# jneem/nnnoiseless

Hardware: AMD Instinct MI355X
Metric: 480-sample frames/sec (whole node) at N concurrent streams (higher is better)
Workload: dtype f32; 1 GPU; configs[2]: 65536 concurrent streams on one GPU, built-in weights.rnn, GRU as batched MFMA GEMM, synthetic 48 kHz sine+noise, 48 frame(s) per stream per step; parity=oracle pinned by the reference's golden pair (built-in model), model=built-in weights.rnn, boundary_format=f32 planar (process_frame's own), streams_per_gpu=65536, streams_total=65536, inputs_ready=True, schedule=stages, lanes=2, parallelism=streams sharded x1, one process per GPU, no data-path collective

## Files before the change

include/nnn_batch.h:

```cpp
#ifndef NNN_BATCH_H
#define NNN_BATCH_H

#include <stddef.h>
#include <stdint.h>

#ifdef __cplusplus
extern "C" {
#endif

typedef struct nnn_batch nnn_batch;
#ifndef RNNOISE_H
typedef struct RNNModel RNNModel;
#endif

#define NNN_FRAME_SIZE 480

RNNModel *nnn_model_from_bytes(const uint8_t *bytes, size_t len);
RNNModel *nnn_model_default(void);
long nnn_convert_rnnoise_text(const char *text, size_t len, uint8_t *out, size_t cap);
RNNModel *nnn_model_from_rnnoise_text(const char *text, size_t len);
void nnn_model_free(RNNModel *m);
RNNModel *nnn_model_clone(const RNNModel *m);
void nnn_model_shape(const RNNModel *m, int32_t shape[12]);

// ... 77 lines not shown
                             const nnn_pcm_layout *layout, void *hip_stream);
int nnn_batch_synthesize_device(nnn_batch *b, const float *d_gains, const float *d_vad, void *d_out, int n_frames,
                                const nnn_pcm_layout *layout, void *hip_stream);
int nnn_batch_analyze_host(nnn_batch *b, const void *in, float *features, int32_t *silence, int n_frames, const nnn_pcm_layout *layout);
int nnn_batch_synthesize_host(nnn_batch *b, const float *gains, const float *vad, void *out, int n_frames, const nnn_pcm_layout *layout);
int nnn_batch_pending_frames(const nnn_batch *b);
int nnn_batch_vad_device(nnn_batch *b, const void *d_in, float *d_vad, int n_frames, const nnn_pcm_layout *layout, void *hip_stream);
int nnn_batch_vad_host(nnn_batch *b, const void *in, float *vad, int n_frames, const nnn_pcm_layout *layout);
int nnn_batch_network_device(nnn_batch *b, const float *d_features, const int32_t *d_silence, float *d_gains, float *d_vad, int n_frames,
                             void *hip_stream);
int nnn_batch_network_host(nnn_batch *b, const float *features, const int32_t *silence, float *gains, float *vad, int n_frames);
int nnn_batch_synchronize(nnn_batch *b);
int nnn_batch_fault(const nnn_batch *b);
int nnn_batch_debug_withhold_flag(nnn_batch *b, int frames_ahead);
int nnn_batch_debug_schedule(nnn_batch *b, int n_frames, int32_t *out, size_t cap);
int nnn_batch_debug_host_plan(nnn_batch *b, int n_frames, const nnn_pcm_layout *layout, int has_vad, int64_t out[8]);

enum nnn_tap {
    NNN_TAP_FILTERED = 0,
    NNN_TAP_XLP,
    NNN_TAP_AC,
    NNN_TAP_LPC2,
    NNN_TAP_XCORR1,
    NNN_TAP_BEST1,
    NNN_TAP_XCORR2C,
    NNN_TAP_PITCH_SEARCH,
    NNN_TAP_PITCH,
    NNN_TAP_PITCH_GAIN,
    NNN_TAP_X,
    NNN_TAP_P,
// ... 40 lines not shown
```

nnnoiseless_amd/_ffi.py:

```python
import ctypes as C
import os

import numpy as np

FRAME_SIZE = 480

TAPS = ["filtered", "xlp", "ac", "lpc2", "xcorr1", "best1", "xcorr2c", "pitch_search", "pitch", "pitch_gain",
        "X", "P", "ex", "ep", "exp", "features", "silence", "g_raw", "g", "vad", "branch"]

BATCH_SYMBOLS = [
    "nnn_model_from_bytes", "nnn_model_default", "nnn_model_free", "nnn_model_clone", "nnn_model_shape",
    "nnn_convert_rnnoise_text", "nnn_model_from_rnnoise_text",
    "nnn_batch_create", "nnn_batch_create_grouped", "nnn_batch_destroy", "nnn_batch_num_streams", "nnn_batch_reset",
    "nnn_batch_process_device", "nnn_batch_process_host", "nnn_batch_process_pcm_device", "nnn_batch_process_pcm_host",
    "nnn_batch_synchronize", "nnn_batch_clone", "nnn_batch_state_bytes", "nnn_batch_save_state", "nnn_batch_load_state",
    "nnn_batch_set_taps", "nnn_batch_set_schedule", "nnn_batch_set_inputs_ready", "nnn_debug_activations",
    "nnn_tap_info", "nnn_batch_read_tap", "nnn_batch_set_profiling", "nnn_batch_num_kernels",
    "nnn_batch_kernel_name", "nnn_batch_read_kernel_times", "nnn_batch_set_graph", "nnn_batch_set_pipeline", "nnn_batch_read_stamps",
    "nnn_host_alloc", "nnn_host_free", "nnn_last_error", "nnn_batch_fault", "nnn_batch_debug_withhold_flag", "nnn_batch_debug_schedule", "nnn_batch_debug_host_plan", "nnn_batch_set_frame_log",
    "nnn_batch_create_opts", "nnn_batch_max_group_frames", "nnn_batch_device_bytes", "nnn_batch_set_back_end", "nnn_device_local_cpulist",
    "nnn_batch_reset_streams", "nnn_batch_export_streams", "nnn_batch_import_streams", "nnn_batch_export_streams_device",
    "nnn_batch_import_streams_device", "nnn_batch_hold_streams", "nnn_batch_resume_streams", "nnn_batch_num_held", "nnn_batch_held_mask",
    "nnn_batch_analyze_device", "nnn_batch_synthesize_device", "nnn_batch_analyze_host", "nnn_batch_synthesize_host", "nnn_batch_pending_frames",
    "nnn_batch_vad_device", "nnn_batch_vad_host", "nnn_batch_network_device", "nnn_batch_network_host",
    "nnn_batch_set_gain_floor", "nnn_batch_get_gain_floor", "nnn_batch_num_floored",
    "nnn_batch_set_channel_link", "nnn_batch_get_channel_link",
]
TRAIN_SYMBOLS = [
    "nnn_train_create", "nnn_train_destroy", "nnn_train_reset", "nnn_train_process_device", "nnn_train_process_host",
]
RESAMPLE_SYMBOLS = [
    "nnn_resampler_create", "nnn_resampler_destroy", "nnn_resampler_reset", "nnn_resampler_max_output",
    "nnn_resampler_process_device", "nnn_resampler_process_host",
]
# ... 155 lines not shown
        L.nnn_batch_set_graph.argtypes = [vp, i32]
        L.nnn_batch_clone.restype = vp
        L.nnn_batch_clone.argtypes = [vp]
        L.nnn_batch_state_bytes.restype = sz
        L.nnn_batch_state_bytes.argtypes = [vp]
        L.nnn_batch_save_state.argtypes = [vp, vp, sz]
        L.nnn_batch_load_state.argtypes = [vp, vp, sz]
        L.nnn_batch_set_taps.argtypes = [vp, i32]
        L.nnn_batch_set_schedule.argtypes = [vp, i32, i32]
        L.nnn_debug_activations.argtypes = [i32, i32, vp, vp, i32]
        L.nnn_batch_set_pipeline.argtypes = [vp, i32]
        L.nnn_batch_set_inputs_ready.argtypes = [vp, i32]
        for name, at in (("nnn_batch_set_frame_log", [vp, vp, sz]), ("nnn_batch_fault", [vp]), ("nnn_batch_debug_withhold_flag", [vp, i32]),
                         ("nnn_batch_debug_schedule", [vp, i32, C.POINTER(C.c_int32), sz]),
                         ("nnn_batch_debug_host_plan", [vp, i32, C.POINTER(PcmLayout), i32, C.POINTER(C.c_int64)]),
                         ("nnn_batch_create_opts", [C.POINTER(vp), C.POINTER(i32), i32, i32, C.POINTER(BatchOpts)]),
                         ("nnn_batch_max_group_frames", [vp]), ("nnn_batch_device_bytes", [vp]), ("nnn_batch_set_back_end", [vp, i32])):
            if hasattr(L, name):
                getattr(L, name).argtypes = at
        if hasattr(L, "nnn_batch_create_opts"):
            L.nnn_batch_create_opts.restype = vp
            L.nnn_batch_device_bytes.restype = sz
        if hasattr(L, "nnn_batch_reset_streams"):
            ip = C.POINTER(i32)
            L.nnn_batch_reset_streams.argtypes = [vp, ip, i32]
            L.nnn_batch_export_streams.argtypes = [vp, ip, i32, vp, sz]
            L.nnn_batch_import_streams.argtypes = [vp, ip, i32, vp, sz]
            L.nnn_batch_export_streams_device.argtypes = [vp, ip, i32, vp, vp]
            L.nnn_batch_import_streams_device.argtypes = [vp, ip, i32, vp, vp]
        if hasattr(L, "nnn_batch_hold_streams"):
# ... 230 lines not shown
```

nnnoiseless_amd/csrc/nnn_batch_core.hip:

```cpp
#pragma once

static thread_local std::string g_err;
static std::recursive_mutex g_rt_mu;
constexpr int MARK_DEVICES = 64;
static std::atomic<uint64_t> g_call_mark[MARK_DEVICES];
static std::atomic<uint64_t> g_next_batch_id{1};
#define NNN_RT_LOCK std::lock_guard<std::recursive_mutex> rt_lock_(g_rt_mu)
extern "C" const char *nnn_last_error(void) { return g_err.c_str(); }
extern "C" int nnn_device_local_cpulist(int device, char *buf, size_t cap)
{
    if (!buf || cap < 2) return 1;
    buf[0] = 0;
    char id[64] = {0};
    if (hipDeviceGetPCIBusId(id, (int)sizeof(id), device) != hipSuccess || !id[0]) return 1;
    for (char *p = id; *p; p++)
        if (*p >= 'A' && *p <= 'F') *p = (char)(*p - 'A' + 'a');
    char path[160];
    snprintf(path, sizeof(path), "/sys/bus/pci/devices/%s/local_cpulist", id);
    FILE *f = fopen(path, "r");
    if (!f) return 1;
    const bool ok = fgets(buf, (int)cap, f) != nullptr;
    fclose(f);
    if (!ok) { buf[0] = 0; return 1; }
    for (char *p = buf; *p; p++)
// ... 37 lines not shown
    const float *vad = nullptr;
};
constexpr int NSTREAMS = 5;
constexpr int EVR = 16;
enum SchedMode { SCHED_SEQ = 0, SCHED_LANES = 1, SCHED_STAGES = 2 };
constexpr int AUTO_BIG = 16384;
constexpr long long HANDOFF_TICKS = 10000ll * 100000ll;

struct Paths {
    int sched = SCHED_LANES;
    bool sched_auto = true;
    int n_lanes = 1;
    int host_chunk = -1;
    int wf_min_g = 0;
    int rnn_rows = 0;
    int hp_split = -1;
    int lpc_head = -1;
    int pitch_chain = 1;
    int hp_tpb = 0;
    int x_rides = -1;
    int lpc_wide = -1;
    int lpc_fc = 0;
    int back_mode = -1;
    bool use_pipeline = true;
    bool inputs_ready = false;
};
static Paths read_paths()
{
    Paths p;
    if (const char *e = knob("NNN_HOST_CHUNK")) p.host_chunk = atoi(e);
    if (const char *e = knob("NNN_RNN_WF_MIN_G")) p.wf_min_g = atoi(e);
    if (const char *e = knob("NNN_HP_SPLIT")) p.hp_split = atoi(e);
    if (const char *e = dev_knob("NNN_HP_TPB")) p.hp_tpb = atoi(e);
    if (const char *e = knob("NNN_LPC_HEAD")) p.lpc_head = atoi(e);
    if (const char *e = dev_knob("NNN_X_RIDES")) p.x_rides = atoi(e);
    if (const char *e = knob("NNN_PITCH_CHAIN")) p.pitch_chain = atoi(e);
    if (const char *e = dev_knob("NNN_LPC_WIDE")) p.lpc_wide = atoi(e);
    if (const char *e = dev_knob("NNN_LPC_FC")) p.lpc_fc = atoi(e);
    if (const char *e = knob("NNN_SCHED")) {
        if (!strcmp(e, "seq")) p.sched = SCHED_SEQ;
        else if (!strcmp(e, "lanes")) p.sched = SCHED_LANES;
        else if (!strcmp(e, "stages")) p.sched = SCHED_STAGES;
        p.sched_auto = false;
    }
    if (const char *e = knob("NNN_LANES")) {
        const int v = atoi(e);
// ... 10 lines not shown
enum BackEnd { BACK_UNFUSED = 0, BACK_RNN_ALONE = 1, BACK_FUSED = 2 };
enum RnnKernel : uint8_t { RK_BACK, RK_WF_BUILTIN, RK_WF_ANY, RK_PLAIN };
struct GroupPlan {
    int g = 0;
    BackEnd back = BACK_UNFUSED;
    int hp = 0;
    bool held = false;
    bool floor = false;
    bool link = false;
    bool head = false;
    bool lpc_in_pitch = false;
    int lpc_fc = 0;
    bool chain = false;
    bool riders = false;
    uint8_t *rnn = nullptr;
};

enum MemKind : uint8_t { MEM_DEVICE, MEM_PINNED, MEM_MAPPED };
template <class T> struct GrowBuf {
    T *p = nullptr;
    size_t cap = 0;
    MemKind kind = MEM_DEVICE;
    int release()
    {
        if (p) HIPCHK(kind == MEM_DEVICE ? hipFree(p) : hipHostFree(p));
        p = nullptr, cap = 0;
        return 0;
    }
    hipError_t alloc(size_t n) { return kind == MEM_DEVICE ? hipMalloc((void **)&p, n) : hipHostMalloc((void **)&p, n, kind == MEM_MAPPED ? hipHostMallocMapped : 0); }
};

struct nnn_batch {
    Buffers b[NSET];
    ModelDims md;
    struct ModelGroup {
        RnnPlan plan;
        const uint4 *wq = nullptr;
        const float *fpar = nullptr;
        size_t rnn_lds = 0;
        bool wf = false;
        bool shape_builtin = false;
        WfPlan wp;
        size_t wf_lds = 0;
        int rows = 32;
        int tile0 = 0, ntiles = 0;
        size_t back_lds = 0, rnn16_lds = 0;
        BkActs acts = {};
        int vad_rows = 0, vad_mb = 0;
        size_t vad_lds = 0;
        int net_rows = 0;
        size_t net_lds = 0;
    };
    Paths paths;
    Paths created;
    GroupPlan plan;
    std::vector<ModelGroup> groups;
    std::vector<RNNModel> models;
    std::vector<int> group_streams;
    int device = 0;
    int S = 0, S_pad = 0, NT = 0;
    uint64_t frame_count = 0;
    int depth = 1;
    int gmax = GROUP;
    int nset = GROUP, nslot = slots_for(GROUP, 1);
    size_t device_bytes = 0;
    uint64_t group_count = 0;
    int last_set = 0;
    std::vector<void *> allocs;
    std::vector<std::pair<void *, size_t>> state_bufs;
    GrowBuf<char> stage;
    GrowBuf<float> stage_vad;
    std::vector<char> stage_host;
    GrowBuf<char> zc_host{nullptr, 0, MEM_MAPPED};
    char *zc_dev = nullptr;
    hipStream_t copy_in = nullptr, copy_out = nullptr;
// ... 128 lines not shown
```

nnnoiseless_amd/csrc/nnn_batch_create.hip:

```cpp
#pragma once

static void make_tables(std::vector<float> &window, std::vector<float> &dct, std::vector<float2> &tw,
                        std::vector<float> &tansig, std::vector<float> &bin_frac, std::vector<int> &bin_band, float &wnorm)
{
    const double pi = 3.14159265358979323846;
    window.resize(WINDOW);
    for (int i = 0; i < FRAME; i++) {
        double s = sin(0.5 * pi * ((double)i + 0.5) / (double)FRAME);
        float w = (float)sin(0.5 * pi * s * s);
        window[i] = w;
        window[WINDOW - 1 - i] = w;
    }
    float acc = 0.0f;
    for (int i = 0; i < WINDOW; i++) acc += window[i] * window[i];
    wnorm = 1.0f / acc;
    dct.resize(NB * NB);
    for (int i = 0; i < NB; i++)
        for (int j = 0; j < NB; j++) {
            float v = (float)cos(((double)i + 0.5) * (double)j * pi / (double)NB);
            if (j == 0) v *= sqrtf(0.5f);
            dct[i * NB + j] = v;
        }
    tw.resize(WINDOW);
    for (int k = 0; k < WINDOW; k++) {
// ... 74 lines not shown
    if (!G.rows) return G;
    while (G.rows > 16 && G.ntiles * (TILE / G.rows) < RNN_SMALL_BATCH_BLOCKS) G.rows /= 2;
    if (paths.rnn_rows && (size_t)rnn_lds(G.plan, paths.rnn_rows).total <= kLdsMax) G.rows = paths.rnn_rows;
    G.rnn_lds = (size_t)rnn_lds(G.plan, G.rows).total;
    for (int half = 2; half >= 1 && !G.vad_rows; half--)
        for (int rows = TILE; rows >= 16 && !G.vad_rows; rows /= 2)
            if ((size_t)vad_lds(vad_plan_view(G.plan), rows).total <= kLdsMax / half && vad_gru_mb(G.plan, rows)) G.vad_rows = rows;
    if (G.vad_rows) {
        G.vad_mb = vad_gru_mb(G.plan, G.vad_rows);
        G.vad_lds = (size_t)vad_lds(vad_plan_view(G.plan), G.vad_rows).total;
    }
    G.net_rows = paths.rnn_rows && (size_t)net_lds(G.plan, paths.rnn_rows).total <= kLdsMax ? paths.rnn_rows : 16;
    G.net_lds = (size_t)net_lds(G.plan, G.net_rows).total;
    G.wp = wf_plan_of(G.plan);
    G.wf_lds = (size_t)wf_lds(G.wp).total;
    {
        constexpr RnnPlan cls = BkShapeBuiltin::plan();
        const bool shape_ok = pl.dense.n == cls.dense.n && pl.vad.n == cls.vad.n && pl.noise.n == cls.noise.n && pl.dn.n == cls.dn.n;
        G.shape_builtin = shape_ok;
        const size_t fb = (size_t)back_lds(G.plan, true).total, rb = (size_t)back_lds(G.plan, false).total;
        G.back_lds = shape_ok && fb <= kLdsMax ? fb : 0;
        G.rnn16_lds = shape_ok && rb <= kLdsMax ? rb : 0;
        G.acts = BkActs{G.plan.dense.act, G.plan.vad.act, G.plan.noise.act, G.plan.dn.act, G.plan.out.act, G.plan.act_vo};
    }
    G.wf = !paths.rnn_rows && G.plan.dense.nb <= 2 && G.plan.vad.nb <= 2 && G.plan.noise.nb <= 3 && G.plan.dn.nb <= 6 && G.plan.vad.rec.ksteps <= WF_KS_REC &&
           G.plan.noise.rec.ksteps <= WF_KS_REC && G.plan.dn.rec.ksteps <= WF_KS_REC && G.wf_lds <= kLdsMax;
    return G;
}

static int create_check_args(nnn_batch *h, const int *group_streams, int n_groups, int device, int gmax, int &n_streams)
{
    h->gmax = gmax < 1 ? 1 : (gmax > GROUP ? GROUP : gmax);
    n_streams = 0;
    for (int g = 0; g < n_groups; g++) {
        if (group_streams[g] <= 0) return fail("group %d: stream count must be positive", g);
        if (g + 1 < n_groups && group_streams[g] % TILE) return fail("group %d: every group but the last must be a multiple of %d streams", g, TILE);
        n_streams += group_streams[g];
    }
    int ndev = 0;
    HIPCHK(hipGetDeviceCount(&ndev));
    if (device < 0 || device >= ndev) return fail("no HIP device %d (found %d)", device, ndev);
    if (device >= MARK_DEVICES) return fail("device %d: the library keeps per-device call marks for devices 0 .. %d only", device, MARK_DEVICES - 1);
    HIPCHK(hipSetDevice(device));
    h->device = device;
    return 0;
}
static int create_streams_and_events(nnn_batch *h)
{
    HIPCHK(hipStreamCreateWithFlags(&h->stream, hipStreamNonBlocking));
    HIPCHK(hipEventCreateWithFlags(&h->ev_in, hipEventDisableTiming));
    HIPCHK(hipEventCreateWithFlags(&h->ev_last, hipEventDisableTiming));
    for (int p = 0; p < 2; p++) {
        for (int s = 0; s < ST_COUNT; s++)
            for (int i = 0; i < EVR; i++) HIPCHK(hipEventCreateWithFlags(&h->ev[p][s][i], hipEventDisableTiming));
        HIPCHK(hipEventCreateWithFlags(&h->ev_done[p], hipEventDisableTiming));
    }
    return 0;
}
static int create_model_groups(nnn_batch *h, const RNNModel *const *models, const int *group_streams, int n_groups, const Paths &paths,
// ... 17 lines not shown
        h->models.push_back(*model);
        RnnPlan plan;
        ModelDims md;
        nnn_model_pack(*model, wqs[g], fpars[g], plan, md);
        delete own;
        nnn_batch::ModelGroup &G = h->groups[g];
        G = plan_model_group(plan, (group_streams[g] + TILE - 1) / TILE, paths);
        if (!G.rows) return fail("model too large for the RNN kernel's LDS operand matrices");
        G.tile0 = tile0;
        tile0 += G.ntiles;
        h->md.nd = md.nd > h->md.nd ? md.nd : h->md.nd;
        h->md.nv = md.nv > h->md.nv ? md.nv : h->md.nv;
        h->md.nn = md.nn > h->md.nn ? md.nn : h->md.nn;
        h->md.ndn = md.ndn > h->md.ndn ? md.ndn : h->md.ndn;
    }
    h->plan.rnn = new uint8_t[n_groups]();
    return 0;
}
static int create_state_arrays(nnn_batch *h)
{
    const size_t Sp = (size_t)h->S_pad;
    const ModelDims &md = h->md;
    Buffers &b = h->b[0];
    memset(&b, 0, sizeof(b));
    b.S = h->S; b.S_pad = h->S_pad; b.NT = h->NT;
    b.nslot = h->nslot;
    b.gru_v_w = md.nv; b.gru_n_w = md.nn; b.gru_dn_w = md.ndn;
    HIPCHK(dalloc(h, &b.hist, Sp * hist_stride(h->nslot), true));
    HIPCHK(dalloc(h, &b.hp_mem, Sp * 2, true));
    HIPCHK(dalloc(h, &b.hp_last, Sp, true));
    HIPCHK(dalloc(h, &b.dec, Sp * dec_len(h->nslot), true));
// ... 213 lines not shown
```

nnnoiseless_amd/csrc/nnn_batch_debug.hip:

```cpp
#pragma once

struct TapDesc { int len; int is_int; int layout;  int sub_ofs; int sub_len; int needs_taps; };
static int last_slot(const nnn_batch *h) { return h ? (int)((h->frame_count + h->nslot - 1) % h->nslot) : 0; }
static bool tap_desc(const nnn_batch *h, int tap, TapDesc &d, const void **ptr)
{
    const Buffers *b = h ? &h->b[h->last_set] : nullptr;
#define TP(field) (b ? (const void *)b->field : nullptr)
    switch (tap) {
    case NNN_TAP_FILTERED: d = {FRAME, 0, 3, 0, FRAME, 0}; *ptr = TP(hist); return true;
    case NNN_TAP_XLP: d = {XLP, 0, 0, 0, XLP, 1}; *ptr = TP(xlp_ti); return true;
    case NNN_TAP_AC: d = {5, 0, 0, last_slot(h) * 10, (h ? h->nslot : 0) * 10, 0}; *ptr = TP(lpc); return true;
    case NNN_TAP_LPC2: d = {5, 0, 0, last_slot(h) * 10 + 5, (h ? h->nslot : 0) * 10, 0}; *ptr = TP(lpc); return true;
    case NNN_TAP_XCORR1: d = {NLAG1, 0, 0, 0, NLAG1, 1}; *ptr = TP(xc1); return true;
    case NNN_TAP_BEST1: d = {2, 1, 0, 0, 2, 1}; *ptr = TP(best1); return true;
    case NNN_TAP_XCORR2C: d = {10, 0, 0, 0, 10, 1}; *ptr = TP(xc2); return true;
    case NNN_TAP_PITCH_SEARCH: d = {1, 1, 0, 0, 1, 1}; *ptr = TP(psearch); return true;
    case NNN_TAP_PITCH: d = {1, 1, 0, 0, 1, 0}; *ptr = TP(pitch); return true;
    case NNN_TAP_PITCH_GAIN: d = {1, 0, 0, 0, 1, 0}; *ptr = TP(pgain); return true;
    case NNN_TAP_X: d = {2 * FREQ, 0, 2, 0, 2 * FREQ, 1}; *ptr = TP(X); return true;
    case NNN_TAP_P: d = {2 * FREQ, 0, 4, 0, 2 * FREQ, 1}; *ptr = TP(P); return true;
    case NNN_TAP_EX: d = {NB, 0, 0, 0, NB, 0}; *ptr = TP(ex); return true;
    case NNN_TAP_EP: d = {NB, 0, 0, 0, NB, 0}; *ptr = TP(ep); return true;
    case NNN_TAP_EXP: d = {NB, 0, 0, 0, NB, 0}; *ptr = TP(exp_); return true;
    case NNN_TAP_FEATURES: d = {NFEAT, 0, 0, 0, NFEAT, 1}; *ptr = TP(feat); return true;
// ... 163 lines not shown
    if (cap < HEAD + PER_NODE * sc.nodes.size()) return fail("schedule buffer too small: %zu entries needed", HEAD + PER_NODE * sc.nodes.size());
    const int32_t head[HEAD] = {(int32_t)sc.nodes.size(), (int32_t)cp.sizes.size(), cp.pipe, cp.sched, cp.lanes, sc.fill, sc.fill_after_done, sc.last_syn};
    memcpy(out, head, sizeof(head));
    out += HEAD;
    for (const Node &n : sc.nodes) {
        const int32_t v[8] = {n.stage, n.group, n.frames, n.first, n.stream, n.first_use, n.record, n.n_waits};
        memcpy(out, v, sizeof(v));
        for (int w = 0; w < MAX_WAITS; w++) {
            const Wait x = w < n.n_waits ? n.waits[w] : Wait{-1, -1, -1};
            out[8 + 3 * w] = x.origin, out[9 + 3 * w] = x.stage, out[10 + 3 * w] = x.group;
        }
        out += PER_NODE;
    }
    return 0;
}
extern "C" int nnn_batch_debug_host_plan(nnn_batch *h, int n_frames, const nnn_pcm_layout *L, int has_vad, int64_t out[8])
{
    if (!h || !out || n_frames < 1) return fail("null argument or no frames");
    if (int rc = check_layout(h, L)) return rc;
    const HostPlan p = plan_host_call(h, n_frames, *L, has_vad != 0);
    const int64_t v[8] = {p.route, p.chunk, p.n_chunks, (int64_t)p.span, (int64_t)p.vbytes, (int64_t)p.vofs, p.drop, p.vad_masked};
    memcpy(out, v, sizeof(v));
    return 0;
}
extern "C" int nnn_batch_set_back_end(nnn_batch *h, int mode)
{
    if (!h) return fail("null batch");
    if (mode < -1 || mode > 4) return fail("unknown back-end mode %d", mode);
    h->paths.back_mode = mode;
    return 0;
}
extern "C" int nnn_batch_set_pipeline(nnn_batch *h, int on)
{
    if (!h) return fail("null batch");
    h->paths.use_pipeline = on != 0;
    return 0;
}
extern "C" int nnn_batch_set_schedule(nnn_batch *h, int mode, int lanes)
{
    if (!h) return fail("null batch");
    if (mode < SCHED_SEQ || mode > SCHED_STAGES) return fail("unknown schedule %d", mode);
    h->paths.sched = mode;
    if (lanes >= 1 && lanes <= NSTREAMS - 1) h->paths.n_lanes = lanes;
    h->paths.sched_auto = false;
    return 0;
}
// ... 1 lines not shown
```

nnnoiseless_amd/csrc/nnn_batch_launch.hip:

```cpp
#pragma once

struct Launcher {
    nnn_batch *h;
    hipStream_t st;
    bool prof;
    template <class K, class... A> void go(int id, K kern, dim3 grid, dim3 block, size_t lds, A... args)
    {
        hipEvent_t e0 = nullptr, e1 = nullptr;
        if (prof) {
            hipEventCreate(&e0);
            hipEventCreate(&e1);
            hipEventRecord(e0, st);
        }
        hipLaunchKernelGGL(kern, grid, block, lds, st, args...);
        if (prof) {
            hipEventRecord(e1, st);
            h->evp.push_back(e0);
            h->evp.push_back(e1);
            h->evp_kernel.push_back(id);
        }
    }
};


static int lpc_launch(const nnn_batch *h, int g)
{
    const Paths &p = h->paths;
    const unsigned NT = (unsigned)h->NT, ug = (unsigned)g;
    if (p.lpc_wide >= 0 ? p.lpc_wide != 0 : NT * ug < 512u) return 0;
    int fc = LPC_FC;
    while (fc > 1 && NT * ((ug + fc - 1) / fc) < 2048u) fc /= 2;
    if (p.lpc_fc > 0) fc = p.lpc_fc < LPC_FC ? p.lpc_fc : LPC_FC;
    return fc;
}
static bool pitch_chained(const nnn_batch *h, int g)
{
    const int pc = h->paths.pitch_chain;
    return pc > 0 && g > 1 && (pc > 1 || (unsigned)h->S_pad / PK_SPB < 1024u);
}

static void plan_group(const nnn_batch *h, int g, GroupPlan &p)
{
    const Paths &k = h->paths;
    p.g = g;
    const int m = k.back_mode >= 0 ? k.back_mode : g > 1 ? 0 : ((h->S_pad <= 8192 && !h->beside_others) ? 1 : 3);
    const bool fused = m == 1 || m == 2, all_g = m == 2 || m == 4;
    p.back = m == 0 || (g > 1 && !all_g) ? BACK_UNFUSED : (fused ? BACK_FUSED : BACK_RNN_ALONE);
    for (const nnn_batch::ModelGroup &G : h->groups)
        if ((fused ? G.back_lds : G.rnn16_lds) == 0) p.back = BACK_UNFUSED;
    const bool split = k.hp_split >= 0 ? k.hp_split != 0 : h->NT <= 256;
    p.hp = !split ? 0 : ((k.hp_tpb ? k.hp_tpb == 2 : (g > 1 && h->NT >= 8)) ? 2 : 1);
    p.floor = h->n_floored > 0;
    p.link = h->link_ch > 1;
    p.held = h->n_held > 0;
    p.lpc_in_pitch = g == 1 && h->S_pad <= (split ? 8192 : 6144) && k.lpc_wide < 0 && k.lpc_fc == 0;
    p.head = p.lpc_in_pitch && split && k.lpc_head != 0;
    p.lpc_fc = p.lpc_in_pitch ? 0 : lpc_launch(h, g);
    p.chain = pitch_chained(h, g);
    p.riders = g == 1 && p.back == BACK_FUSED && (k.x_rides >= 0 ? k.x_rides != 0 : h->S_pad <= 8192);
    for (size_t i = 0; i < h->groups.size(); i++) {
        const nnn_batch::ModelGroup &G = h->groups[i];
        const int min_g = k.wf_min_g > 0 ? k.wf_min_g : ((G.ntiles * (TILE / WF_ROWS) >= 1024 || h->beside_others) ? 2 : 1);
        p.rnn[i] = p.back == BACK_RNN_ALONE ? RK_BACK : !(G.wf && g >= min_g) ? RK_PLAIN : G.shape_builtin ? RK_WF_BUILTIN : RK_WF_ANY;
    }
}

using RnnWfKernel = decltype(&k_rnn_wf<WfShapeAny>);
using BackKernel = decltype(&k_back<true, BkShapeBuiltin>);
using RnnPlainKernel = decltype(&k_rnn<false>);
static const RnnPlainKernel kRnnKernels[2] = {k_rnn<false>, k_rnn<true>};
static const auto kVadKernel = &k_vad;
static const auto kNetKernel = &k_net;
static const RnnWfKernel kRnnWfKernels[2] = {k_rnn_wf<WfShapeAny>, k_rnn_wf<BkShapeBuiltin>};
#define NNN_BK(F, XR, HELD, FLOOR) {k_back<F, BkShapeBuiltin, XR, HELD, FLOOR, false>, k_back<F, BkShapeBuiltin, XR, HELD, FLOOR, true>}
static const BackKernel kBackFused[2][2][2][2] = {
    {{NNN_BK(true, false, false, false), NNN_BK(true, false, false, true)}, {NNN_BK(true, false, true, false), NNN_BK(true, false, true, true)}},
    {{NNN_BK(true, true, false, false), NNN_BK(true, true, false, true)}, {NNN_BK(true, true, true, false), NNN_BK(true, true, true, true)}}};
static const BackKernel kBackRnnAlone[2][2][2] = {
    {NNN_BK(false, false, false, false), NNN_BK(false, false, false, true)},
    {NNN_BK(false, false, true, false), NNN_BK(false, false, true, true)}};
#undef NNN_BK
static std::vector<const void *> big_lds_kernels()
{
    std::vector<const void *> v;
    for (RnnPlainKernel k : kRnnKernels) v.push_back((const void *)k);
    for (RnnWfKernel k : kRnnWfKernels) v.push_back((const void *)k);
    for (const auto &by_held : kBackFused)
        for (const auto &by_floor : by_held)
            for (const auto &by_link : by_floor)
                for (BackKernel k : by_link) v.push_back((const void *)k);
    for (const auto &by_floor : kBackRnnAlone)
        for (const auto &by_link : by_floor)
            for (BackKernel k : by_link) v.push_back((const void *)k);
    v.push_back((const void *)kVadKernel);
    v.push_back((const void *)kNetKernel);
    return v;
}

static void launch_stage(nnn_batch *h, int s, int set0, const GroupPlan &p, const StepParams *sp0, hipStream_t st, bool prof, bool plain_out, const StepParams *call = nullptr, int fill = 0,
                         const SplitIo *io = nullptr)
{
// ... 25 lines not shown
    }
    case ST_FFT:
        if (p.back == BACK_FUSED) {
            for (const nnn_batch::ModelGroup &G : h->groups)
                L.go(K_BACK, kBackFused[p.riders][p.held][p.floor][p.link], dim3((unsigned)(G.ntiles * (TILE / BK_ROWS))), dim3(BK_T), G.back_lds, b, sp0, G.acts, G.wq, G.fpar, G.tile0, g);
            break;
        }
        L.go(K_FFT_XP, k_fft_xp, dim3(Sp * ug / FFT_SPB), dim3(64 * FFT_SPB), 0, b, sp0, g);
        break;
    case ST_RNN:
        if (p.back == BACK_FUSED) break;
        for (size_t i = 0; i < h->groups.size(); i++) {
            const nnn_batch::ModelGroup &G = h->groups[i];
            if (p.rnn[i] == RK_BACK)
                L.go(K_RNN, kBackRnnAlone[p.held][p.floor][p.link], dim3((unsigned)(G.ntiles * (TILE / BK_ROWS))), dim3(BK_T), G.rnn16_lds, b, sp0, G.acts, G.wq, G.fpar, G.tile0, g);
            else if (p.rnn[i] == RK_WF_BUILTIN || p.rnn[i] == RK_WF_ANY)
                L.go(K_RNN, kRnnWfKernels[p.rnn[i] == RK_WF_BUILTIN], dim3((unsigned)(G.ntiles * (TILE / WF_ROWS))), dim3(64 * WF_WAVES), G.wf_lds, b, G.plan, G.wp,
                     G.wq, G.fpar, G.tile0, g);
            else
                L.go(K_RNN, kRnnKernels[p.link], dim3((unsigned)(G.ntiles * (TILE / G.rows))), dim3(64 * RNN_WAVES), G.rnn_lds, b, G.plan, G.wq, G.fpar,
                     G.tile0, G.rows, g);
        }
        break;
    case ST_SYN:
        if (p.back == BACK_FUSED) break;
        if (plain_out) L.go(K_SYNTH, k_synth<true>, dim3(Sp / FFT_SPB), dim3(64 * FFT_SPB), 0, b, sp0, g);
        else L.go(K_SYNTH, k_synth<false>, dim3(Sp / FFT_SPB), dim3(64 * FFT_SPB), 0, b, sp0, g);
        break;
    case ST_FEAT:
        hipLaunchKernelGGL(k_features, dim3(NT), dim3(64 * FEAT_WAVES), 0, st, b, g);
// ... 289 lines not shown
```

nnnoiseless_amd/csrc/nnn_rnn_wf.hip:

```cpp
#pragma once

namespace nnn {

constexpr int WF_ROWS = 16, WF_WAVES = 12, WF_FS_W = 72;

struct WfGru {
    f32x4 acc[3][2];
    float zz[4], sold[4];
};
constexpr int WF_KS_REC = 3;
struct WfWeights {
    Frags<2, WF_KS_REC> zr;
    Frags<1, WF_KS_REC> h;
    float bias[3];
};
__device__ __forceinline__ void wf_load_weights(WfWeights &w, const LayerDesc &L, const uint4 *__restrict__ Wq, const float *__restrict__ fpar,
                                                int nbi, int lane)
{
    const uint4 *Brec = Wq + L.rec.wofs + (size_t)nbi * 3 * L.rec.ksteps * 64;
    load_frags<2, 0, WF_KS_REC>(w.zr, L.rec, Brec, lane);
    load_frags<1, 2, WF_KS_REC>(w.h, L.rec, Brec, lane);
    const int neuron = nbi * 16 + (lane & 15);
#pragma unroll
    for (int g = 0; g < 3; g++) w.bias[g] = neuron < L.n ? fpar[L.bias + g * L.n + neuron] : 0.0f;
// ... 396 lines not shown
        }
        NNN_STAMPW(b, 33 + 5 * srole, t == 2 && srole >= 0);
#if defined(NNN_STAMPS) && NNN_WFSTAMP_PHASE == 2
        NNN_STAMPW(b, 14 + wave0, t == 2);
#endif
        lds_barrier();
        NNN_STAMPW(b, 34 + 5 * srole, t == 2 && srole >= 0);
    }
    gru_state_io<T>(pl.vad, rm, sv, SPv, wp.sw_v, false);
    gru_state_io<T>(pl.noise, rm, sn, SPn, wp.sw_n, false);
    gru_state_io<T>(pl.dn, rm, sdn, SPdn, wp.sw_dn, false);
    if (wave0 == WF_WAVES - 1 && rowl) NNN_TI(b.mem_id, 1, tile, trow)[0] = mem_id;
    NNN_STAMP(b, 52);
}

}
```

Baseline: 75.54 million frames/s.

## Chain several row sets per workgroup in the wavefront RNN kernel

Adds k_rnn_wfc, a variant of the wavefront GRU kernel where each workgroup processes up to four 16-row sets back to back. The next set's GRU state and cepstral ring are prefetched into a second LDS buffer while the current set runs, so the pipeline fill and drain cost and the weight-fragment loads are paid once per chain rather than once per set. It is selected automatically for the built-in shape when g>=8 and there are at least two tiles per CU. The cost is about 158 KiB of LDS per workgroup and four times fewer workgroups, which lowers occupancy and parallelism.

```diff
diff --git a/include/nnn_batch.h b/include/nnn_batch.h
--- a/include/nnn_batch.h
+++ b/include/nnn_batch.h
@@ -115,6 +115,9 @@
 int nnn_batch_fault(const nnn_batch *b);
 int nnn_batch_debug_withhold_flag(nnn_batch *b, int frames_ahead);
 int nnn_batch_debug_schedule(nnn_batch *b, int n_frames, int32_t *out, size_t cap);
+int nnn_debug_rnn_chain(int n_streams, int n_cus, int g, int lds_total, int knob);
+int nnn_batch_debug_rnn_plan(nnn_batch *b, int g, int32_t *out, size_t cap);
+int nnn_batch_set_rnn_chain(nnn_batch *b, int sets);
 int nnn_batch_debug_host_plan(nnn_batch *b, int n_frames, const nnn_pcm_layout *layout, int has_vad, int64_t out[8]);
 
 enum nnn_tap {
diff --git a/nnnoiseless_amd/_ffi.py b/nnnoiseless_amd/_ffi.py
--- a/nnnoiseless_amd/_ffi.py
+++ b/nnnoiseless_amd/_ffi.py
@@ -18,6 +18,7 @@
     "nnn_tap_info", "nnn_batch_read_tap", "nnn_batch_set_profiling", "nnn_batch_num_kernels",
     "nnn_batch_kernel_name", "nnn_batch_read_kernel_times", "nnn_batch_set_graph", "nnn_batch_set_pipeline", "nnn_batch_read_stamps",
     "nnn_host_alloc", "nnn_host_free", "nnn_last_error", "nnn_batch_fault", "nnn_batch_debug_withhold_flag", "nnn_batch_debug_schedule", "nnn_batch_debug_host_plan", "nnn_batch_set_frame_log",
+    "nnn_debug_rnn_chain", "nnn_batch_debug_rnn_plan", "nnn_batch_set_rnn_chain",
     "nnn_batch_create_opts", "nnn_batch_max_group_frames", "nnn_batch_device_bytes", "nnn_batch_set_back_end", "nnn_device_local_cpulist",
     "nnn_batch_reset_streams", "nnn_batch_export_streams", "nnn_batch_import_streams", "nnn_batch_export_streams_device",
     "nnn_batch_import_streams_device", "nnn_batch_hold_streams", "nnn_batch_resume_streams", "nnn_batch_num_held", "nnn_batch_held_mask",
@@ -203,6 +204,7 @@
         for name, at in (("nnn_batch_set_frame_log", [vp, vp, sz]), ("nnn_batch_fault", [vp]), ("nnn_batch_debug_withhold_flag", [vp, i32]),
                          ("nnn_batch_debug_schedule", [vp, i32, C.POINTER(C.c_int32), sz]),
                          ("nnn_batch_debug_host_plan", [vp, i32, C.POINTER(PcmLayout), i32, C.POINTER(C.c_int64)]),
+                         ("nnn_debug_rnn_chain", [i32, i32, i32, i32, i32]), ("nnn_batch_debug_rnn_plan", [vp, i32, C.POINTER(C.c_int32), sz]), ("nnn_batch_set_rnn_chain", [vp, i32]),
                          ("nnn_batch_create_opts", [C.POINTER(vp), C.POINTER(i32), i32, i32, C.POINTER(BatchOpts)]),
                          ("nnn_batch_max_group_frames", [vp]), ("nnn_batch_device_bytes", [vp]), ("nnn_batch_set_back_end", [vp, i32])):
             if hasattr(L, name):
diff --git a/nnnoiseless_amd/csrc/nnn_batch_core.hip b/nnnoiseless_amd/csrc/nnn_batch_core.hip
--- a/nnnoiseless_amd/csrc/nnn_batch_core.hip
+++ b/nnnoiseless_amd/csrc/nnn_batch_core.hip
@@ -75,6 +75,7 @@
     int host_chunk = -1;
     int wf_min_g = 0;
     int rnn_rows = 0;
+    int rnn_chain = -1;
     int hp_split = -1;
     int lpc_head = -1;
     int pitch_chain = 1;
@@ -91,6 +92,10 @@
     Paths p;
     if (const char *e = knob("NNN_HOST_CHUNK")) p.host_chunk = atoi(e);
     if (const char *e = knob("NNN_RNN_WF_MIN_G")) p.wf_min_g = atoi(e);
+    if (const char *e = dev_knob("NNN_RNN_CHAIN")) {
+        const int v = atoi(e);
+        if (v == 0 || v == 1 || v == 2 || v == 4) p.rnn_chain = v ? v : 1;
+    }
     if (const char *e = knob("NNN_HP_SPLIT")) p.hp_split = atoi(e);
     if (const char *e = dev_knob("NNN_HP_TPB")) p.hp_tpb = atoi(e);
     if (const char *e = knob("NNN_LPC_HEAD")) p.lpc_head = atoi(e);
@@ -131,6 +136,7 @@
     bool chain = false;
     bool riders = false;
     uint8_t *rnn = nullptr;
+    uint8_t *rnn_c = nullptr;
 };
 
 enum MemKind : uint8_t { MEM_DEVICE, MEM_PINNED, MEM_MAPPED };
@@ -159,6 +165,7 @@
         bool shape_builtin = false;
         WfPlan wp;
         size_t wf_lds = 0;
+        size_t wfc_lds = 0;
         int rows = 32;
         int tile0 = 0, ntiles = 0;
         size_t back_lds = 0, rnn16_lds = 0;
@@ -176,6 +183,7 @@
     std::vector<int> group_streams;
     int device = 0;
     int S = 0, S_pad = 0, NT = 0;
+    int n_cus = 256;
     uint64_t frame_count = 0;
     int depth = 1;
     int gmax = GROUP;
diff --git a/nnnoiseless_amd/csrc/nnn_batch_create.hip b/nnnoiseless_amd/csrc/nnn_batch_create.hip
--- a/nnnoiseless_amd/csrc/nnn_batch_create.hip
+++ b/nnnoiseless_amd/csrc/nnn_batch_create.hip
@@ -112,6 +112,7 @@
     G.net_lds = (size_t)net_lds(G.plan, G.net_rows).total;
     G.wp = wf_plan_of(G.plan);
     G.wf_lds = (size_t)wf_lds(G.wp).total;
+    G.wfc_lds = (size_t)wfc_lds(G.wp).total;
     {
         constexpr RnnPlan cls = BkShapeBuiltin::plan();
         const bool shape_ok = pl.dense.n == cls.dense.n && pl.vad.n == cls.vad.n && pl.noise.n == cls.noise.n && pl.dn.n == cls.dn.n;
@@ -141,6 +142,9 @@
     if (device >= MARK_DEVICES) return fail("device %d: the library keeps per-device call marks for devices 0 .. %d only", device, MARK_DEVICES - 1);
     HIPCHK(hipSetDevice(device));
     h->device = device;
+#ifdef __HIPCC__
+    HIPCHK(hipDeviceGetAttribute(&h->n_cus, hipDeviceAttributeMultiprocessorCount, device));
+#endif
     return 0;
 }
 static int create_streams_and_events(nnn_batch *h)
@@ -188,7 +192,8 @@
         h->md.nn = md.nn > h->md.nn ? md.nn : h->md.nn;
         h->md.ndn = md.ndn > h->md.ndn ? md.ndn : h->md.ndn;
     }
-    h->plan.rnn = new uint8_t[n_groups]();
+    h->plan.rnn = new uint8_t[2 * n_groups]();
+    h->plan.rnn_c = h->plan.rnn + n_groups;
     return 0;
 }
 static int create_state_arrays(nnn_batch *h)
diff --git a/nnnoiseless_amd/csrc/nnn_batch_debug.hip b/nnnoiseless_amd/csrc/nnn_batch_debug.hip
--- a/nnnoiseless_amd/csrc/nnn_batch_debug.hip
+++ b/nnnoiseless_amd/csrc/nnn_batch_debug.hip
@@ -201,6 +201,30 @@
     }
     return 0;
 }
+extern "C" int nnn_debug_rnn_chain(int n_streams, int n_cus, int g, int lds_total, int knob)
+{
+    if (n_streams < 1 || n_cus < 1 || g < 1) return 0;
+    const int streams = (n_streams + TILE - 1) / TILE * TILE;
+    return rnn_chain_of(streams, n_cus, g, lds_total > 0 ? lds_total : wfc_lds(wf_plan_of(BkShapeBuiltin::plan())).total, knob == 0 ? 1 : knob);
+}
+extern "C" int nnn_batch_debug_rnn_plan(nnn_batch *h, int g, int32_t *out, size_t cap)
+{
+    if (!h || !out) return fail("null argument");
+    if (g < 1 || g > h->gmax) return fail("g must be 1 .. %d", h->gmax);
+    if (cap < 4 * h->groups.size()) return fail("plan buffer too small: %zu entries needed", 4 * h->groups.size());
+    GroupPlan p = h->plan;
+    plan_group(h, g, p);
+    for (size_t i = 0; i < h->groups.size(); i++) {
+        const nnn_batch::ModelGroup &G = h->groups[i];
+        const bool wf = p.back != BACK_FUSED && (p.rnn[i] == RK_WF_BUILTIN || p.rnn[i] == RK_WF_ANY);
+        const int c = wf ? p.rnn_c[i] : 0;
+        out[4 * i] = p.back == BACK_FUSED ? -1 : p.rnn[i];
+        out[4 * i + 1] = c;
+        out[4 * i + 2] = wf ? G.ntiles * (TILE / WF_ROWS) / c : 0;
+        out[4 * i + 3] = wf ? (int32_t)(c > 1 ? G.wfc_lds : G.wf_lds) : 0;
+    }
+    return 0;
+}
 extern "C" int nnn_batch_debug_host_plan(nnn_batch *h, int n_frames, const nnn_pcm_layout *L, int has_vad, int64_t out[8])
 {
     if (!h || !out || n_frames < 1) return fail("null argument or no frames");
@@ -217,6 +241,13 @@
     h->paths.back_mode = mode;
     return 0;
 }
+extern "C" int nnn_batch_set_rnn_chain(nnn_batch *h, int sets)
+{
+    if (!h) return fail("null batch");
+    if (sets != -1 && sets != 0 && sets != 1 && sets != 2 && sets != 4) return fail("rnn chain must be -1, 0, 1, 2 or 4, not %d", sets);
+    h->paths.rnn_chain = sets == 0 ? 1 : sets;
+    return 0;
+}
 extern "C" int nnn_batch_set_pipeline(nnn_batch *h, int on)
 {
     if (!h) return fail("null batch");
diff --git a/nnnoiseless_amd/csrc/nnn_batch_launch.hip b/nnnoiseless_amd/csrc/nnn_batch_launch.hip
--- a/nnnoiseless_amd/csrc/nnn_batch_launch.hip
+++ b/nnnoiseless_amd/csrc/nnn_batch_launch.hip
@@ -37,6 +37,14 @@
 {
     const int pc = h->paths.pitch_chain;
     return pc > 0 && g > 1 && (pc > 1 || (unsigned)h->S_pad / PK_SPB < 1024u);
+}
+
+static int rnn_chain_of(int streams, int n_cus, int g, int lds_total, int knob)
+{
+    constexpr int min_per_cu = 2;
+    if (knob == 1 || g < WFC_MIN_G || lds_total > WFC_LDS_MAX) return 1;
+    if (knob == 2 || knob == 4) return knob;
+    return streams / TILE >= min_per_cu * n_cus ? 4 : 1;
 }
 
 static void plan_group(const nnn_batch *h, int g, GroupPlan &p)
@@ -62,6 +70,7 @@
         const nnn_batch::ModelGroup &G = h->groups[i];
         const int min_g = k.wf_min_g > 0 ? k.wf_min_g : ((G.ntiles * (TILE / WF_ROWS) >= 1024 || h->beside_others) ? 2 : 1);
         p.rnn[i] = p.back == BACK_RNN_ALONE ? RK_BACK : !(G.wf && g >= min_g) ? RK_PLAIN : G.shape_builtin ? RK_WF_BUILTIN : RK_WF_ANY;
+        p.rnn_c[i] = p.rnn[i] == RK_WF_BUILTIN ? (uint8_t)rnn_chain_of(G.ntiles * TILE, h->n_cus, g, (int)G.wfc_lds, k.rnn_chain) : 1;
     }
 }
 
@@ -72,6 +81,7 @@
 static const auto kVadKernel = &k_vad;
 static const auto kNetKernel = &k_net;
 static const RnnWfKernel kRnnWfKernels[2] = {k_rnn_wf<WfShapeAny>, k_rnn_wf<BkShapeBuiltin>};
+static const auto kRnnWfcKernel = &k_rnn_wfc<BkShapeBuiltin>;
 #define NNN_BK(F, XR, HELD, FLOOR) {k_back<F, BkShapeBuiltin, XR, HELD, FLOOR, false>, k_back<F, BkShapeBuiltin, XR, HELD, FLOOR, true>}
 static const BackKernel kBackFused[2][2][2][2] = {
     {{NNN_BK(true, false, false, false), NNN_BK(true, false, false, true)}, {NNN_BK(true, false, true, false), NNN_BK(true, false, true, true)}},
@@ -85,6 +95,7 @@
     std::vector<const void *> v;
     for (RnnPlainKernel k : kRnnKernels) v.push_back((const void *)k);
     for (RnnWfKernel k : kRnnWfKernels) v.push_back((const void *)k);
+    v.push_back((const void *)kRnnWfcKernel);
     for (const auto &by_held : kBackFused)
         for (const auto &by_floor : by_held)
             for (const auto &by_link : by_floor)
@@ -140,6 +151,9 @@
             const nnn_batch::ModelGroup &G = h->groups[i];
             if (p.rnn[i] == RK_BACK)
                 L.go(K_RNN, kBackRnnAlone[p.held][p.floor][p.link], dim3((unsigned)(G.ntiles * (TILE / BK_ROWS))), dim3(BK_T), G.rnn16_lds, b, sp0, G.acts, G.wq, G.fpar, G.tile0, g);
+            else if (p.rnn[i] == RK_WF_BUILTIN && p.rnn_c[i] > 1)
+                L.go(K_RNN, kRnnWfcKernel, dim3((unsigned)(G.ntiles * (TILE / WF_ROWS) / p.rnn_c[i])), dim3(64 * WF_WAVES), G.wfc_lds, b, G.plan,
+                     G.wp, G.wq, G.fpar, G.tile0, g, (int)p.rnn_c[i]);
             else if (p.rnn[i] == RK_WF_BUILTIN || p.rnn[i] == RK_WF_ANY)
                 L.go(K_RNN, kRnnWfKernels[p.rnn[i] == RK_WF_BUILTIN], dim3((unsigned)(G.ntiles * (TILE / WF_ROWS))), dim3(64 * WF_WAVES), G.wf_lds, b, G.plan, G.wp,
                      G.wq, G.fpar, G.tile0, g);
diff --git a/nnnoiseless_amd/csrc/nnn_rnn_wf.hip b/nnnoiseless_amd/csrc/nnn_rnn_wf.hip
--- a/nnnoiseless_amd/csrc/nnn_rnn_wf.hip
+++ b/nnnoiseless_amd/csrc/nnn_rnn_wf.hip
@@ -434,4 +434,266 @@
     NNN_STAMP(b, 52);
 }
 
-}
+struct WfcLds { WfLds o; int SPv1, SPn1, SPdn1, crs1, dc1, total; };
+__host__ __device__ constexpr WfcLds wfc_lds(const WfPlan &w)
+{
+    constexpr int plane3 = 3 * WF_ROWS * 2;
+    WfcLds c{};
+    c.o = wf_lds(w);
+    int at = c.o.total;
+    c.SPv1 = lds_take(at, plane3 * w.sw_v);
+    c.SPn1 = lds_take(at, plane3 * w.sw_n);
+    c.SPdn1 = lds_take(at, plane3 * w.sw_dn);
+    c.crs1 = lds_take(at, CEPS_MEM * NB * WF_ROWS * 4);
+    c.dc1 = lds_take(at, 28 * WF_ROWS * 4);
+    c.total = at;
+    return c;
+}
+static_assert(wfc_lds(wf_plan_of(BkShapeBuiltin::plan())).total == 161536, "k_rnn_wfc's LDS for the built-in shape class");
+constexpr int WFC_LDS_MAX = 160 * 1024;
+static_assert(wfc_lds(wf_plan_of(BkShapeBuiltin::plan())).total <= WFC_LDS_MAX, "... fits");
+constexpr int WFC_MIN_G = 8;
+
+template <class SH>
+__global__ void __launch_bounds__(64 * WF_WAVES, NNN_WF_MINWAVES) k_rnn_wfc(Buffers b, RnnPlan pl_rt, WfPlan wp_rt, const uint4 *__restrict__ Wq,
+                                                             const float *__restrict__ fpar, int tile0, int g, int c)
+{
+    RnnPlan pl = pl_rt;
+    WfPlan wp = wp_rt;
+    if constexpr (WfFixed<SH>::value) {
+        constexpr RnnPlan p0 = SH::plan();
+        constexpr WfPlan w0 = wf_plan_of(p0);
+        pl = p0;
+        pl.dense.act = pl_rt.dense.act; pl.vad.act = pl_rt.vad.act; pl.noise.act = pl_rt.noise.act; pl.dn.act = pl_rt.dn.act;
+        pl.out.act = pl_rt.out.act; pl.act_vo = pl_rt.act_vo;
+        wp = w0;
+    }
+    HIP_DYNAMIC_SHARED(float, lds_raw)
+    constexpr int rm = WF_ROWS;
+    const int wave0 = __builtin_amdgcn_readfirstlane((int)(threadIdx.x >> 6));
+    const int lane0 = threadIdx.x & 63;
+    int wave = wave0, lane = lane0;
+    int tile, rfirst;
+    rnn_block_rows(b, tile0, rm * c, tile, rfirst);
+    int list = 0, N = 0;
+    for (int i = 0; i < c; i++) {
+        const int r = rfirst + rm * i;
+        if (tile * TILE + r < b.S && live_any(b, tile, r, rm)) list |= (r / rm) << (2 * N++);
+    }
+    if (N == 0) return;
+    auto r0_of = [&](int s) { return ((list >> (2 * s)) & 3) * rm; };
+    const int G = N * g;
+    const bool rowl = lane0 < rm;
+    const WfcLds oc = wfc_lds(wp);
+    const WfLds o = oc.o;
+    auto planes = [&](int at) { return (unsigned short *)(lds_raw + at / 4); };
+    float *tab = lds_raw + o.tab / 4;
+    int *live = (int *)(lds_raw + o.live / 4);
+    unsigned short *Xv = planes(o.Xv), *Xn = planes(o.Xn), *Xdn = planes(o.Xdn);
+    unsigned short *RSv = planes(o.RSv), *RSn = planes(o.RSn), *RSdn = planes(o.RSdn);
+    unsigned short *FS = planes(o.FS);
+    float *cnb = lds_raw + o.cnb / 4;
+    auto SPv_of = [&](int s) { return planes((s & 1) ? oc.SPv1 : o.SPv); };
+    auto SPn_of = [&](int s) { return planes((s & 1) ? oc.SPn1 : o.SPn); };
+    auto SPdn_of = [&](int s) { return planes((s & 1) ? oc.SPdn1 : o.SPdn); };
+    auto crs_of = [&](int s) { return lds_raw + ((s & 1) ? oc.crs1 : o.crs) / 4; };
+    auto dc_of = [&](int s) { return lds_raw + ((s & 1) ? oc.dc1 : o.dc) / 4; };
+    const int cD = pl.dense.out_col, cV = pl.cV, cF = pl.cF;
+    constexpr int T = 64 * WF_WAVES;
+    auto states_io = [&](int s, bool load) {
+        const int r0 = r0_of(s);
+        gru_state_io<T>(pl.vad, rm, b.gru_v + ((size_t)tile * TILE * b.gru_v_w + (size_t)r0 * pl.vad.n), SPv_of(s), wp.sw_v, load);
+        gru_state_io<T>(pl.noise, rm, b.gru_n + ((size_t)tile * TILE * b.gru_n_w + (size_t)r0 * pl.noise.n), SPn_of(s), wp.sw_n, load);
+        gru_state_io<T>(pl.dn, rm, b.gru_dn + ((size_t)tile * TILE * b.gru_dn_w + (size_t)r0 * pl.dn.n), SPdn_of(s), wp.sw_dn, load);
+    };
+    static_assert(2 * T >= WF_ROWS * 96 && T >= WF_ROWS * 48, "WfcStage: values per thread");
+    struct WfcStage { float v[4]; };
+    auto states_get = [&](int s, WfcStage &st, int tid) {
+        const int r0 = r0_of(s);
+        const float *sv = b.gru_v + ((size_t)tile * TILE * b.gru_v_w + (size_t)r0 * pl.vad.n), *sn = b.gru_n + ((size_t)tile * TILE * b.gru_n_w + (size_t)r0 * pl.noise.n),
+                    *sdn = b.gru_dn + ((size_t)tile * TILE * b.gru_dn_w + (size_t)r0 * pl.dn.n);
+        st.v[0] = tid < rm * pl.dn.n ? sdn[tid] : 0.0f;
+        st.v[1] = tid + T < rm * pl.dn.n ? sdn[tid + T] : 0.0f;
+        st.v[2] = tid < rm * pl.noise.n ? sn[tid] : 0.0f;
+        st.v[3] = tid < rm * pl.vad.n ? sv[tid] : 0.0f;
+    };
+    auto state_put = [&](const LayerDesc &L, unsigned short *SP, int sw, int e, float v) {
+        const int row = e / L.n, col = e - row * L.n;
+        if (e < rm * L.n) store_split(SP, rm * sw, row * sw + col, v);
+    };
+    auto states_put = [&](int s, const WfcStage &st, int tid) {
+        state_put(pl.dn, SPdn_of(s), wp.sw_dn, tid, st.v[0]);
+        state_put(pl.dn, SPdn_of(s), wp.sw_dn, tid + T, st.v[1]);
+        state_put(pl.noise, SPn_of(s), wp.sw_n, tid, st.v[2]);
+        state_put(pl.vad, SPv_of(s), wp.sw_v, tid, st.v[3]);
+    };
+    auto state_back = [&](const LayerDesc &L, const unsigned short *SP, int sw, float *state, int ln) {
+        for (int e = ln; e < rm * L.n; e += 64) {
+            const int row = e / L.n, col = e - row * L.n;
+            state[e] = load_split(SP, rm * sw, row * sw + col);
+        }
+    };
+    constexpr int RING = CEPS_MEM * NB * WF_ROWS;
+    static_assert(4 * T >= RING, "WfcStage: values per thread");
+    auto ring_get = [&](int s, WfcStage &st, int tid) {
+        const float *cm = NNN_TI(b.ceps_mem, CEPS_MEM * NB, tile, r0_of(s) + (tid & (rm - 1)));
+#pragma unroll
+        for (int i = 0; i < 4; i++) st.v[i] = tid + i * T < RING ? cm[(size_t)((tid + i * T) / rm) * TILE] : 0.0f;
+    };
+    auto ring_put = [&](int s, const WfcStage &st, int tid) {
+        float *crs = crs_of(s);
+#pragma unroll
+        for (int i = 0; i < 4; i++)
+            if (tid + i * T < RING) crs[tid + i * T] = st.v[i];
+    };
+    auto pair_dists = [&](int s, int wv, int ln) {
+        float *crs = crs_of(s), *dc = dc_of(s);
+        if (ln < rm)
+            for (int p = wv; p < 28; p += WF_WAVES) dc[p * rm + ln] = pair_dist(crs, p, ln, rm);
+    };
+    {
+        uint4 *z = (uint4 *)Xv;
+        const int n16 = (o.crs - o.Xv) / 16;
+        for (int i = (int)threadIdx.x; i < n16; i += T) z[i] = make_uint4(0u, 0u, 0u, 0u);
+        uint4 *z1 = (uint4 *)planes(oc.SPv1);
+        const int m16 = (oc.crs1 - oc.SPv1) / 16;
+        for (int i = (int)threadIdx.x; i < m16; i += T) z1[i] = make_uint4(0u, 0u, 0u, 0u);
+        for (int i = (int)threadIdx.x; i < 201; i += T) tab[i] = b.tansig[i];
+        WfcStage st;
+        ring_get(0, st, (int)threadIdx.x);
+        ring_put(0, st, (int)threadIdx.x);
+    }
+    lds_barrier();
+    states_io(0, true);
+    pair_dists(0, wave, lane);
+    int mem_id = wave == WF_WAVES - 1 ? NNN_TI(b.mem_id, 1, tile, r0_of(0) + (lane & 15))[0] : 0;
+    int mem_next = 0;
+    const int W_N = 6, W_V = 9, W_F = 11;
+    WfWeights wts;
+    if (wave < W_N) wf_load_weights(wts, pl.dn, Wq, fpar, wave < pl.dn.nb ? wave : 0, lane);
+    else if (wave < W_V) wf_load_weights(wts, pl.noise, Wq, fpar, wave - W_N < pl.noise.nb ? wave - W_N : 0, lane);
+    else if (wave < W_F) wf_load_weights(wts, pl.vad, Wq, fpar, wave - W_V < pl.vad.nb ? wave - W_V : 0, lane);
+    else wf_load_weights(wts, pl.vad, Wq, fpar, 0, lane);
+    lds_barrier();
+    WfGru ua;
+    if (wave == WF_WAVES - 1) wf_features_load(wts, b, 0, tile, r0_of(0), lane);
+    if (wave0 == WF_WAVES - 1) wf_setprio_high();
+    auto set_of = [&](int cf) { return (cf >= g ? 1 : 0) + (cf >= 2 * g ? 1 : 0) + (cf >= 3 * g ? 1 : 0); };
+    for (int t = -1; t < G + 3; t++) {
+        lane = launder_v(lane0);
+        wave = launder_s(wave0);
+        const int cv = t, cn = t - 1, cd = t - 2, co = t - 3, cf = t + 1;
+        const bool on_v = cv >= 0 && cv < G, on_n = cn >= 0 && cn < G, on_d = cd >= 0 && cd < G, on_o = co >= 0 && co < G, on_f = cf >= 0 && cf < G;
+        const int sv_ = set_of(cv), sn_ = set_of(cn), sd_ = set_of(cd), so_ = set_of(co), sf_ = set_of(cf);
+        unsigned short *Xn_n = Xn + (cn & 1) * 3 * rm * wp.w_n;
+        unsigned short *Xdn_d = Xdn + ((cd + 3) % 3) * 3 * rm * wp.w_dn;
+        if (wave < W_N) {
+            if (on_d && wave < pl.dn.nb) wf_gru_a(pl.dn, Xdn_d, wp.w_dn, SPdn_of(sd_), RSdn, wp.sw_dn, Wq, wts, tab, wave, lane, ua);
+        } else if (wave < W_V) {
+            if (on_n && wave - W_N < pl.noise.nb) wf_gru_a(pl.noise, Xn_n - cV, wp.w_n, SPn_of(sn_), RSn, wp.sw_n, Wq, wts, tab, wave - W_N, lane, ua);
+        } else if (wave < W_F) {
+            WfDenseW<3> dw;
+            const bool mine_o = on_o && wave - W_V < pl.out.nb;
+            if (on_v && wave - W_V < pl.vad.nb) wf_gru_a(pl.vad, Xv - cD, wp.w_v, SPv_of(sv_), RSv, wp.sw_v, Wq, wts, tab, wave - W_V, lane, ua);
+            if (mine_o) {
+                const int *lv = live + 16 * (co & 7);
+                const int fo = co - so_ * g, r0 = r0_of(so_);
+                wf_dense_load(dw, pl.out, Wq, fpar, wave - W_V, lane);
+                wf_dense<true>(pl.out, SPdn_of(so_), wp.sw_dn, Wq, dw, tab, wave - W_V, lane, [&](int lrow, int band, const float (&v)[4]) {
+                    if (b.link) {
+                        rnn_gain_out4(b, fo, tile, r0 + lrow, band, lv + lrow, v);
+                    } else {
+#pragma unroll
+                        for (int q = 0; q < 4; q++) rnn_gain_out(b, fo, tile, r0 + lrow + q, band, lv[lrow + q] != 0, v[q]);
+                    }
+                });
+            }
+        } else {
+            if (on_f) {
+                const int ff = cf - sf_ * g, r0 = r0_of(sf_);
+                if (ff == 0 && sf_ > 0) {
+                    if (rowl) NNN_TI(b.mem_id, 1, tile, r0_of(sf_ - 1) + lane)[0] = mem_id;
+                    mem_id = mem_next;
+                }
+                wf_features(b, wf_features_in(wts), ff, tile, r0, lane, crs_of(sf_), dc_of(sf_), cnb, FS, live + 16 * (cf & 7), mem_id);
+            }
+            if (cf + 1 >= 0 && cf + 1 < G) {
+                const int s1 = set_of(cf + 1), f1 = cf + 1 - s1 * g, r1 = r0_of(s1);
+                wf_features_load(wts, b, f1, tile, r1, lane);
+                if (f1 == 0 && s1 > 0) mem_next = NNN_TI(b.mem_id, 1, tile, r1 + (lane & 15))[0];
+            }
+        }
+        lds_barrier();
+        const int kv = cv - sv_ * g, tid = 64 * wave + lane;
+        const bool next_set = on_v && sv_ + 1 < N;
+        WfcStage stage;
+        if (next_set && kv == 3) states_get(sv_ + 1, stage, tid);
+        if (next_set && kv == 4) ring_get(sv_ + 1, stage, tid);
+        if (wave < W_N) {
+            WfDenseW<2> dw;
+            const bool mine_d = on_f && wave < pl.dense.nb;
+            if (on_d && wave < pl.dn.nb) {
+                unsigned short *SPd = SPdn_of(sd_);
+                wf_gru_b(pl.dn, RSdn, wp.sw_dn, Wq, wts, tab, live + 16 * (cd & 7), wave, lane, ua,
+                         [&](int row, int n, float v) { store_split(SPd, rm * wp.sw_dn, row * wp.sw_dn + n, v); });
+            }
+            if (mine_d) {
+                unsigned short *Xnn = Xn + (cf & 1) * 3 * rm * wp.w_n;
+                wf_dense_load(dw, pl.dense, Wq, fpar, wave, lane);
+                wf_dense(pl.dense, FS - cF, WF_FS_W, Wq, dw, tab, wave, lane, [&](int row, int n, float v) {
+                    store_split(Xv, rm * wp.w_v, row * wp.w_v + n, v);
+                    store_split(Xnn, rm * wp.w_n, row * wp.w_n + (cD - cV) + n, v);
+                });
+            }
+        } else if (wave < W_V) {
+            if (on_n && wave - W_N < pl.noise.nb) {
+                unsigned short *Xd = Xdn + (cn % 3) * 3 * rm * wp.w_dn, *SPs = SPn_of(sn_);
+                wf_gru_b(pl.noise, RSn, wp.sw_n, Wq, wts, tab, live + 16 * (cn & 7), wave - W_N, lane, ua, [&](int row, int n, float v) {
+                    store_split(SPs, rm * wp.sw_n, row * wp.sw_n + n, v);
+                    store_split(Xd, rm * wp.w_dn, row * wp.w_dn + n, v);
+                });
+            }
+            if (on_f) {
+                unsigned short *Xnn = Xn + (cf & 1) * 3 * rm * wp.w_n, *Xd = Xdn + (cf % 3) * 3 * rm * wp.w_dn;
+                for (int i = 64 * (wave - W_N) + lane; i < 3 * rm * 6; i += 64 * (W_V - W_N)) {
+                    const int plx = i / (rm * 6), rem = i - plx * rm * 6, row = rem / 6, c8 = rem - row * 6;
+                    const uint4 v = *(const uint4 *)(FS + (size_t)plx * rm * WF_FS_W + row * WF_FS_W + 8 * c8);
+                    *(uint4 *)(Xnn + (size_t)plx * rm * wp.w_n + row * wp.w_n + (cF - cV) + 8 * c8) = v;
+                    *(uint4 *)(Xd + (size_t)plx * rm * wp.w_dn + row * wp.w_dn + cF + 8 * c8) = v;
+                }
+            }
+        } else if (wave < W_F) {
+            if (on_v && wave - W_V < pl.vad.nb) {
+                unsigned short *Xnn = Xn + (cv & 1) * 3 * rm * wp.w_n, *Xd = Xdn + (cv % 3) * 3 * rm * wp.w_dn, *SPs = SPv_of(sv_);
+                wf_gru_b(pl.vad, RSv, wp.sw_v, Wq, wts, tab, live + 16 * (cv & 7), wave - W_V, lane, ua, [&](int row, int n, float v) {
+                    store_split(SPs, rm * wp.sw_v, row * wp.sw_v + n, v);
+                    store_split(Xnn, rm * wp.w_n, row * wp.w_n + n, v);
+                    store_split(Xd, rm * wp.w_dn, row * wp.w_dn + cV + n, v);
+                });
+            }
+        } else {
+            if (on_n && rowl) {
+                const unsigned short *Xv1 = Xn + (cn & 1) * 3 * rm * wp.w_n;
+                NNN_TIF(b, vad, 1, cn - sn_ * g, tile, r0_of(sn_) + lane)[0] =
+                    rnn_vad_out(pl, fpar, Xv1, rm * wp.w_n, wp.w_n, 0, lane, live + 16 * (cn & 7), tab);
+            }
+            if (on_v && sv_ > 0 && (kv == 1 || kv == 2)) {
+                const int r0 = r0_of(sv_ - 1);
+                if (kv == 1) {
+                    state_back(pl.vad, SPv_of(sv_ - 1), wp.sw_v, b.gru_v + ((size_t)tile * TILE * b.gru_v_w + (size_t)r0 * pl.vad.n), lane);
+                    state_back(pl.noise, SPn_of(sv_ - 1), wp.sw_n, b.gru_n + ((size_t)tile * TILE * b.gru_n_w + (size_t)r0 * pl.noise.n), lane);
+                } else {
+                    state_back(pl.dn, SPdn_of(sv_ - 1), wp.sw_dn, b.gru_dn + ((size_t)tile * TILE * b.gru_dn_w + (size_t)r0 * pl.dn.n), lane);
+                }
+            }
+        }
+        if (next_set && kv == 3) states_put(sv_ + 1, stage, tid);
+        if (next_set && kv == 4) ring_put(sv_ + 1, stage, tid);
+        if (next_set && kv == 5) pair_dists(sv_ + 1, wave, lane);
+        lds_barrier();
+    }
+    states_io(N - 1, false);
+    if (wave0 == WF_WAVES - 1 && rowl) NNN_TI(b.mem_id, 1, tile, r0_of(N - 1) + lane0)[0] = mem_id;
+}
+
+}
```

Result: no change. 75.98 million frames/s (median of 5 runs) (+0.6%).
